# millardjn/rusty_sr

Measured on AMD Instinct MI355X. Metric: output megapixels/sec at 3x upscale (BASELINE '4x'; reference factor is hard-wired 3), higher is better.
Workload: dtype f32; 1 GPU; 1920x1080 RGB x3 upscale per GPU, imagenet.rsr, rgba8 in/out resident in HBM; io=rgba8, factor=3, parallelism=rowband1, precision=f32

## Files before the change

### rusty_sr_amd/csrc/sr_kernels.hip

```cpp
#include <hip/hip_runtime.h>
#include <stddef.h>
#include <stdint.h>

#include <mutex>
#include <set>
#include <type_traits>
#include <utility>

#include "sr_kernels.h"

#pragma clang fp contract(off)

typedef float f32x2 __attribute__((ext_vector_type(2)));
struct f32p { float x, y; };
__device__ __forceinline__ f32p operator+(f32p a, f32p b) { return f32p{a.x + b.x, a.y + b.y}; }
__device__ __forceinline__ f32p operator-(f32p a, f32p b) { return f32p{a.x - b.x, a.y - b.y}; }
__device__ __forceinline__ f32p operator*(f32p a, f32p b) { return f32p{a.x * b.x, a.y * b.y}; }
__device__ __forceinline__ f32p p_fma(f32p a, f32p b, f32p c) { return f32p{__builtin_fmaf(a.x, b.x, c.x), __builtin_fmaf(a.y, b.y, c.y)}; }
__device__ __forceinline__ void store_map8(char* p, uint32_t a, uint32_t b) { *(uint2*)p = make_uint2(a, b); }
typedef float f32x4 __attribute__((ext_vector_type(4)));
typedef float f32x16 __attribute__((ext_vector_type(16)));
typedef _Float16 f16x8 __attribute__((ext_vector_type(8)));
typedef _Float16 f16x2 __attribute__((ext_vector_type(2)));

template <int PREC>
constexpr bool kPlanar = PREC == 1;
template <int PREC, bool FINAL>
constexpr bool kH16 = PREC == 1 && !FINAL;

namespace {

constexpr int kThreads = 256;
constexpr int kTW = 32;
constexpr int kChunkFloats = 1024;
constexpr int kRingSlots = 5;
constexpr int kRingAhead = 4;
constexpr int kRingBytes = kRingSlots * 4096;

__device__ __forceinline__ float belu(float v, float beta) {
    return __fadd_rn(__fadd_rn(__fmul_rn(beta, v), __builtin_amdgcn_sqrtf(__fadd_rn(__fmul_rn(v, v), 1.0f))), -1.0f);
}

__device__ __forceinline__ f32x2 belu2(f32x2 v, float beta) {
    const f32x2 one = {1.0f, 1.0f};
    const f32x2 t = v * v + one;
    const f32x2 s = {__builtin_amdgcn_sqrtf(t.x), __builtin_amdgcn_sqrtf(t.y)};
    const f32x2 b = {beta, beta};
    return (b * v + s) - one;
}

__device__ __forceinline__ f32p split_value(f32p accm, f32p accx) {
    return p_fma(accx, f32p{1.0f / 2048.0f, 1.0f / 2048.0f}, accm);
}
__device__ __forceinline__ f32p belu2_fused2(f32p v, f32p beta) {
    const f32p one = {1.0f, 1.0f};
    const f32p t = p_fma(v, v, one);
    const f32p s = {__builtin_amdgcn_sqrtf(t.x), __builtin_amdgcn_sqrtf(t.y)};
    return p_fma(beta, v, s) - one;
}

__device__ __forceinline__ void store_belu_tile(float* base, const f32x16& acc, float bias, float beta) {
#pragma unroll
    for (int r = 0; r < 16; r += 2) {
        const f32x2 bb = {bias, bias};
        const f32x2 o = belu2(f32x2{acc[r], acc[r + 1]} + bb, beta);
        const int row = (r & 3) + 8 * (r >> 2);
        base[row * 32] = o.x;
        base[(row + 1) * 32] = o.y;
    }
}

__device__ __forceinline__ void store_belu_tile_lds(float* grow, float* stage, const f32x16& acc, float bias, float beta, int lane) {
    float* sp = stage + (4 * (lane >> 5)) * 32 + (lane & 31);
#pragma unroll
    for (int r = 0; r < 16; r += 2) {
        const f32x2 bb = {bias, bias};
        const f32x2 o = belu2(f32x2{acc[r], acc[r + 1]} + bb, beta);
        const int row = (r & 3) + 8 * (r >> 2);
        sp[row * 32] = o.x;
        sp[(row + 1) * 32] = o.y;
    }
    const f32x4* lp = (const f32x4*)stage + lane;
    const f32x4 v0 = lp[0], v1 = lp[64], v2 = lp[128], v3 = lp[192];
    f32x4* gp = (f32x4*)grow + lane;
    gp[0] = v0; gp[64] = v1; gp[128] = v2; gp[192] = v3;
}

__device__ __forceinline__ int xcd_remap(int bid, int nblk) {
    const int q = nblk >> 3, r = nblk & 7, xcd = bid & 7, idx = bid >> 3;
    return (xcd < r ? xcd * (q + 1) : r * (q + 1) + (xcd - r) * q) + idx;
}

__device__ __forceinline__ int tile_div(int t, TileDiv d) {
    return (int)((__umulhi((uint32_t)t, d.m) + (uint32_t)t) >> d.s);
}

__device__ __forceinline__ void tile_coords(const TileGrid& g, int tiles_x, int t, int& n, int& tx, int& ty) {
    const int tpi = tiles_x * g.tiles_y;
    n = tile_div(t, g.div_tpi);
    const int r = t - n * tpi;
    if (g.bw == 0) {
        ty = tile_div(r, g.div_tx);
        tx = r - ty * tiles_x;
    } else {
        int b = tile_div(r, g.div_blk);
        if (b > g.nfull) b = g.nfull;
        const int rr = r - b * g.bw * g.tiles_y;
        const bool full = b < g.nfull;
        const int w = full ? g.bw : tiles_x - g.nfull * g.bw;
        ty = full ? tile_div(rr, g.div_bw) : tile_div(rr, g.div_rem);
        tx = b * g.bw + (rr - ty * w);
    }
}

__device__ __forceinline__ float load_img(const void* img, int img_ch, bool u8, size_t px, int c) {
    if (u8) return __fdiv_rn((float)((const uint8_t*)img)[px * img_ch + c], 255.0f);
    return ((const float*)img)[px * 3 + c];
}

constexpr float kLoScale = 2048.0f;
typedef __fp16 fp16x2_t __attribute__((ext_vector_type(2)));

__device__ __forceinline__ void split_half2(f32p v, uint32_t& hi2, uint32_t& lo2) {
    const fp16x2_t h = __builtin_amdgcn_cvt_pkrtz(v.x, v.y);
    const f32p hf = {(float)h.x, (float)h.y};
    const f32p r = (v - hf) * f32p{kLoScale, kLoScale};
    hi2 = __builtin_bit_cast(uint32_t, h);
    lo2 = __builtin_bit_cast(uint32_t, __builtin_amdgcn_cvt_pkrtz(r.x, r.y));
}

typedef unsigned short u16x2 __attribute__((ext_vector_type(2)));
__device__ __forceinline__ void domain_track(uint32_t& dom, uint32_t hi2) {
    dom = __builtin_bit_cast(uint32_t, __builtin_elementwise_max(__builtin_bit_cast(u16x2, dom), __builtin_bit_cast(u16x2, hi2 & 0x7fff7fffu)));
}
__device__ __forceinline__ void domain_report(uint32_t dom, int* flag) {
    if (((dom & 0xffffu) >= 0x7bffu) | ((dom >> 16) >= 0x7bffu)) *(volatile int*)flag = 1;
}

__device__ __forceinline__ void store_belu_tile_split_cr(char* base, const f32x16& accm, const f32x16& accx, const f32x4 (&beta)[4], bool write,
                                                         long group_stride, long lo_off, uint32_t& dom) {
#pragma unroll
    for (int j = 0; j < 4; ++j) {
        const int r = 4 * j;
        const f32p v01 = belu2_fused2(split_value(f32p{accm[r], accm[r + 1]}, f32p{accx[r], accx[r + 1]}), f32p{beta[j][0], beta[j][1]});
        const f32p v23 = belu2_fused2(split_value(f32p{accm[r + 2], accm[r + 3]}, f32p{accx[r + 2], accx[r + 3]}), f32p{beta[j][2], beta[j][3]});
        uint32_t h01, l01, h23, l23;
        split_half2(v01, h01, l01);
        split_half2(v23, h23, l23);
        domain_track(dom, h01);
        domain_track(dom, h23);
        if (write) {
            store_map8(base + j * group_stride, h01, h23);
            store_map8(base + j * group_stride + lo_off, l01, l23);
        }
    }
}

template <typename F>
__device__ __forceinline__ void for_each_acc_row(F&& f) {
#pragma unroll
    for (int r = 0; r < 16; ++r) f(r, (r & 3) + 8 * (r >> 2));
}

}

__device__ __forceinline__ const char* uniform_ptr(const void* p) {
    const uint64_t v = (uint64_t)(uintptr_t)p;
    const uint32_t lo = __builtin_amdgcn_readfirstlane((uint32_t)v), hi = __builtin_amdgcn_readfirstlane((uint32_t)(v >> 32));
    return (const char*)(uintptr_t)(((uint64_t)hi << 32) | lo);
}

template <int TH, bool IMG_U8>
__global__ __launch_bounds__(kThreads, 2) void conv0_kernel(Conv0Args a) {
    constexpr int T = TH / 4;
    constexpr int TWH = kTW + 4, THH = TH + 4, NPIX = THH * TWH;
    __shared__ __attribute__((aligned(16))) float s_x[NPIX * 3 + 16];
    __shared__ __attribute__((aligned(16))) float s_w[5 * 8 * 64];

    const int tid = threadIdx.x, lane = tid & 63;
    const int wave = __builtin_amdgcn_readfirstlane(tid >> 6);
    const int i = lane & 31, h = lane >> 5;
    const int tiles_per_img = a.tiles_x * a.tiles_y;
    for (int k = tid; k < 5 * 8 * 64; k += kThreads) s_w[k] = a.wpack[k];
    if (tid < 16) s_x[NPIX * 3 + tid] = 0.f;
    if (blockIdx.x == 0 && tid < 40) a.queue_reset[tid] = (a.queue_grid[tid >> 3] - (tid & 7) + 7) >> 3;
    __shared__ float s_lut[256];
    if constexpr (IMG_U8) s_lut[tid] = __fdiv_rn((float)tid, 255.0f);
    const float bias = a.bias[i], beta = a.beta[i];
  for (int bid = blockIdx.x; bid < a.n_tiles; bid += gridDim.x) {
    const int n = tile_div(bid, a.div_tpi), t = bid - n * tiles_per_img;
    const int ty = tile_div(t, a.div_tx), tx = t - ty * a.tiles_x;
    const int x0 = tx * kTW, y0 = a.y_begin + ty * TH;
    const size_t img_px0 = (size_t)n * a.H * a.W;

    __syncthreads();
    for (int p = tid; p < NPIX; p += kThreads) {
        const int py = p / TWH, px = p - py * TWH;
        const int gy = y0 - 2 + py, gx = x0 - 2 + px;
        f32x4 v = {0.f, 0.f, 0.f, 0.f};
        if (gy >= 0 && gy < a.H && gx >= 0 && gx < a.W) {
            const size_t gp = img_px0 + (size_t)gy * a.W + gx;
            if constexpr (IMG_U8) {
                const uint8_t* q = (const uint8_t*)a.img + gp * a.img_ch;
                v.x = s_lut[q[0]]; v.y = s_lut[q[1]]; v.z = s_lut[q[2]];
            } else {
                v.x = load_img(a.img, a.img_ch, false, gp, 0);
                v.y = load_img(a.img, a.img_ch, false, gp, 1);
                v.z = load_img(a.img, a.img_ch, false, gp, 2);
            }
        }
        s_x[p * 3] = v.x; s_x[p * 3 + 1] = v.y; s_x[p * 3 + 2] = v.z;
    }
    __syncthreads();

    f32x16 acc[T];
#pragma unroll
    for (int m = 0; m < T; ++m)
#pragma unroll
        for (int r = 0; r < 16; ++r) acc[m][r] = 0.f;

    const float* xa = s_x + ((wave * T) * TWH + i) * 3 + h;
    const float* wb = s_w + (h * 32 + i) * 2;
#pragma unroll
    for (int ky = 0; ky < 5; ++ky) {
#pragma unroll
        for (int jj = 0; jj < 4; ++jj) {
            const f32x2 b = *(const f32x2*)(wb + (ky * 4 + jj) * 128);
#pragma unroll
            for (int m = 0; m < T; ++m) {
                const float* row = xa + (m + ky) * TWH * 3;
                acc[m] = __builtin_amdgcn_mfma_f32_32x32x2f32(row[4 * jj], b.x, acc[m], 0, 0, 0);
                const float a2 = (jj == 3 && h) ? 0.0f : row[4 * jj + 2];
                acc[m] = __builtin_amdgcn_mfma_f32_32x32x2f32(a2, b.y, acc[m], 0, 0, 0);
            }
        }
    }

    const bool full_x = x0 + kTW <= a.W;
#pragma unroll
    for (int m = 0; m < T; ++m) {
        const int y = y0 + wave * T + m;
        if (y >= a.y_end) continue;
        float* base = a.dst + ((size_t)n * a.img_stride + (long)y * a.pitch + x0 + 4 * h) * 32 + i;
        if (full_x) {
            store_belu_tile(base, acc[m], bias, beta);
        } else {
            for_each_acc_row([&](int r, int row) {
                if (x0 + 4 * h + row < a.W) base[row * 32] = belu(__fadd_rn(acc[m][r], bias), beta);
            });
        }
    }
  }
}

template <int TH, bool IMG_U8>
__global__ __launch_bounds__(kThreads, 3) void conv0_split_kernel(Conv0Args a) {
    constexpr int T = TH / 4;
    constexpr int TWH = kTW + 4, THH = TH + 4, NPIX = THH * TWH;
    constexpr int NB = 7;
    __shared__ __attribute__((aligned(16))) uint32_t s_px[2][NPIX * 2];
    __shared__ uint32_t s_lut[256];
    const int tid = threadIdx.x, lane = tid & 63;
    const int wave = __builtin_amdgcn_readfirstlane(tid >> 6);
    const int i = lane & 31, h = lane >> 5;
    const int tiles_per_img = a.tiles_x * a.tiles_y;
    if (blockIdx.x == 0 && tid < 40) a.queue_reset[tid] = (a.queue_grid[tid >> 3] - (tid & 7) + 7) >> 3;
    if constexpr (IMG_U8) {
        uint32_t hi2, lo2;
        split_half2(f32p{__fdiv_rn((float)tid, 255.0f), 0.0f}, hi2, lo2);
        s_lut[tid] = (hi2 & 0xffffu) | (lo2 << 16);
    }
    __shared__ __attribute__((aligned(16))) f16x8 s_w[NB * 2 * 64];
    for (int k = tid; k < NB * 2 * 64; k += kThreads) s_w[k] = ((const f16x8*)a.wpack_split)[k];
    const f16x8* wl = s_w + h * 32 + i;
    uint32_t off_a[NB], off_b[NB];
#pragma unroll
    for (int b = 0; b < NB; ++b) {
        const int ta = min(4 * b + 2 * h, 24), tb = min(4 * b + 2 * h + 1, 24);
        off_a[b] = (uint32_t)(((ta / 5) * TWH + ta % 5) * 8);
        off_b[b] = (uint32_t)(((tb / 5) * TWH + tb % 5) * 8);
    }
    const char* abase = (const char*)&s_px[0][0] + ((wave * T) * TWH + i) * 8;
    constexpr uint32_t LO = NPIX * 2 * 4;
    f32x4 bias4[4], beta4[4];
#pragma unroll
    for (int j = 0; j < 4; ++j) {
        bias4[j] = *(const f32x4*)(a.bias + 8 * j + 4 * h);
        beta4[j] = *(const f32x4*)(a.beta + 8 * j + 4 * h);
    }
    uint32_t dom = 0;
    for (int bid = blockIdx.x; bid < a.n_tiles; bid += gridDim.x) {
        const int n = tile_div(bid, a.div_tpi), t = bid - n * tiles_per_img;
        const int ty = tile_div(t, a.div_tx), tx = t - ty * a.tiles_x;
        const int x0 = tx * kTW, y0 = a.y_begin + ty * TH;
        const size_t img_px0 = (size_t)n * a.H * a.W;
        __syncthreads();
        for (int p = tid; p < NPIX; p += kThreads) {
            const int py = p / TWH, px = p - py * TWH;
            const int gy = y0 - 2 + py, gx = x0 - 2 + px;
            uint32_t h0 = 0, h1 = 0, l0 = 0, l1 = 0;
            if (gy >= 0 && gy < a.H && gx >= 0 && gx < a.W) {
                const size_t gp = img_px0 + (size_t)gy * a.W + gx;
                if constexpr (IMG_U8) {
                    const uint8_t* q = (const uint8_t*)a.img + gp * a.img_ch;
                    const uint32_t wr = s_lut[q[0]], wg = s_lut[q[1]], wb = s_lut[q[2]];
                    h0 = __builtin_amdgcn_perm(wg, wr, 0x05040100u); l0 = __builtin_amdgcn_perm(wg, wr, 0x07060302u);
                    h1 = wb & 0xffffu; l1 = wb >> 16;
                } else {
                    const float* q = (const float*)a.img + gp * 3;
                    split_half2(f32p{q[0], q[1]}, h0, l0);
                    split_half2(f32p{q[2], 0.0f}, h1, l1);
                    domain_track(dom, h0);
                    domain_track(dom, h1);
                }
            }
            *(uint2*)&s_px[0][p * 2] = make_uint2(h0, h1);
            *(uint2*)&s_px[1][p * 2] = make_uint2(l0, l1);
        }
        __syncthreads();

        f32x16 accm[T], accx[T];
#pragma unroll
        for (int m = 0; m < T; ++m)
#pragma unroll
            for (int r = 0; r < 16; ++r) { accm[m][r] = bias4[r >> 2][r & 3]; accx[m][r] = 0.f; }
#pragma unroll
        for (int b = 0; b < NB; ++b) {
            const f16x8 bh = wl[(b * 2 + 0) * 64], bl = wl[(b * 2 + 1) * 64];
#pragma unroll
            for (int m = 0; m < T; ++m) {
                const char* ra = abase + off_a[b] + m * TWH * 8;
                const char* rb = abase + off_b[b] + m * TWH * 8;
                const uint2 ha = *(const uint2*)ra, hb2 = *(const uint2*)rb;
                const uint2 la = *(const uint2*)(ra + LO), lb2 = *(const uint2*)(rb + LO);
                const uint32_t ahw[4] = {ha.x, ha.y, hb2.x, hb2.y}, alw[4] = {la.x, la.y, lb2.x, lb2.y};
                const f16x8 ah = __builtin_bit_cast(f16x8, ahw), al = __builtin_bit_cast(f16x8, alw);
                accm[m] = __builtin_amdgcn_mfma_f32_32x32x16_f16(bh, ah, accm[m], 0, 0, 0);
                accx[m] = __builtin_amdgcn_mfma_f32_32x32x16_f16(bl, ah, accx[m], 0, 0, 0);
                accx[m] = __builtin_amdgcn_mfma_f32_32x32x16_f16(bh, al, accx[m], 0, 0, 0);
            }
        }

        const bool full_x = x0 + kTW <= a.W;
#pragma unroll
        for (int m = 0; m < T; ++m) {
            const int y = y0 + wave * T + m;
            if (y >= a.y_end) continue;
            char* base = (char*)(a.dst + ((size_t)n * a.img_stride + (long)y * a.pitch) * 32) + (size_t)(x0 + i) * 16 + 8 * h;
            store_belu_tile_split_cr(base, accm[m], accx[m], beta4, full_x || x0 + i < a.W, (long)a.pitch * 16, (long)a.pitch * 64, dom);
        }
    }
    domain_report(dom, a.domain);
}

template <int TH, int KS>
struct TileGeom {
    static constexpr int R = KS / 2;
    static constexpr int TWH = kTW + 2 * R;
    static constexpr int THH = TH + 2 * R;
    static constexpr int NPIX = THH * TWH;
    static constexpr int NG = (NPIX + 63) / 64;
    static constexpr int PLANE = NG * 64 * 16;
};

template <int IMM>
__device__ __forceinline__ void lds_dma16(const void* base, uint32_t voff, uint32_t lds) {
    asm volatile("s_mov_b32 m0, %0\n\ts_nop 3\n\tglobal_load_lds_dwordx4 %1, %2 offset:%3"
                 :: "s"(lds), "v"(voff), "s"(base), "n"(IMM) : "memory");
}
__device__ __forceinline__ void lds_dma16_at(const void* base, uint32_t byte_off, uint32_t voff, uint32_t lds) {
    const uint64_t b = (uint64_t)(uintptr_t)base;
    asm volatile("s_add_u32 vcc_lo, %0, %2\n\ts_addc_u32 vcc_hi, %1, 0\n\ts_mov_b32 m0, %3\n\ts_nop 0\n\tglobal_load_lds_dwordx4 %4, vcc offset:0"
                 :: "s"((uint32_t)b), "s"((uint32_t)(b >> 32)), "s"(__builtin_amdgcn_readfirstlane(byte_off)), "s"(__builtin_amdgcn_readfirstlane(lds)), "v"(voff)
                 : "vcc", "scc", "memory");
}
__device__ __forceinline__ uint32_t lds_addr(const void* p) {
    return (uint32_t)(uintptr_t)(const __attribute__((address_space(3))) char*)p;
}

template <int TH, int KS, int NW = 4>
struct TileOffsets {
    using G = TileGeom<TH, KS>;
    static constexpr int N = (G::NG + NW - 1) / NW;
    uint32_t v[N];
    template <int PREC>
    __device__ __forceinline__ void init(int pitch, int wave, int lane) {
#pragma unroll
        for (int gi = 0; gi < N; ++gi) {
            const int P = min((wave + NW * gi) * 64 + lane, G::NPIX - 1);
            const int prow = P / G::TWH, pcol = P - prow * G::TWH;
            v[gi] = kPlanar<PREC> ? (uint32_t)(prow * pitch) * 128u + (uint32_t)pcol * 16u : (uint32_t)(prow * pitch + pcol) * 128u;
        }
    }
};

template <int TH, int KS, int PREC, int NW = 4>
__device__ __forceinline__ void stage_tile(char* tile, const float* __restrict__ src, const TileOffsets<TH, KS, NW>& off,
                                           long img_stride, int pitch, int n, int y0, int x0, int wave, int ) {
    using G = TileGeom<TH, KS>;
    const char* origin = kPlanar<PREC> ? uniform_ptr((const char*)(src + ((size_t)n * img_stride + (long)(y0 - G::R) * pitch) * 32) + (long)(x0 - G::R) * 16)
                                       : uniform_ptr(src + ((size_t)n * img_stride + (long)(y0 - G::R) * pitch + (x0 - G::R)) * 32);
#pragma unroll
    for (int gi = 0; gi < TileOffsets<TH, KS, NW>::N; ++gi) {
        const int g = wave + NW * gi;
        if (g < G::NG) {
            const uint32_t dst = __builtin_amdgcn_readfirstlane(lds_addr(tile) + g * 1024);
            if constexpr (kPlanar<PREC>) {
#pragma unroll
                for (int c = 0; c < 8; ++c) lds_dma16_at(origin, (uint32_t)(c * pitch * 16), off.v[gi], dst + c * G::PLANE);
            } else {
#define SR_DMA16(c) lds_dma16<(c) * 16>(origin, off.v[gi], dst + (c) * (G::PLANE - 16))
                SR_DMA16(0); SR_DMA16(1); SR_DMA16(2); SR_DMA16(3); SR_DMA16(4); SR_DMA16(5); SR_DMA16(6); SR_DMA16(7);
#undef SR_DMA16
            }
        }
    }
}

__device__ __forceinline__ void weight_chunk_async(char* ring_slot, const float* __restrict__ chunk,
                                                   int wave, int lane) {
    lds_dma16<0>(uniform_ptr((const char*)chunk + wave * 1024), (uint32_t)(lane * 16),
                 __builtin_amdgcn_readfirstlane(lds_addr(ring_slot) + wave * 1024));
}

template <int PENDING>
__device__ __forceinline__ void ring_barrier() {
    static_assert(PENDING >= 0 && PENDING <= 3, "");
    if constexpr (PENDING == 3) asm volatile("s_waitcnt vmcnt(3) lgkmcnt(0)" ::: "memory");
    else if constexpr (PENDING == 2) asm volatile("s_waitcnt vmcnt(2) lgkmcnt(0)" ::: "memory");
    else if constexpr (PENDING == 1) asm volatile("s_waitcnt vmcnt(1) lgkmcnt(0)" ::: "memory");
    else asm volatile("s_waitcnt vmcnt(0) lgkmcnt(0)" ::: "memory");
    __builtin_amdgcn_s_barrier();
    asm volatile("" ::: "memory");
}

__device__ __forceinline__ void ring_request(char* ring, const float* __restrict__ wpack, int gtap, int slot,
                                             int ntaps_total, int wave, int lane) {
    if (gtap + kRingAhead < ntaps_total) {
        int s2 = slot + kRingAhead;
        if (s2 >= kRingSlots) s2 -= kRingSlots;
        weight_chunk_async(ring + s2 * 4096, wpack + (size_t)(gtap + kRingAhead) * kChunkFloats, wave, lane);
    }
}
template <int EXTRA = 0>
__device__ __forceinline__ void ring_advance(int& gtap, int& slot, int ntaps_total) {
    const int pending = max(0, min(kRingAhead - 1 - EXTRA, ntaps_total - 2 - EXTRA - gtap));
    ++gtap;
    slot = slot == kRingSlots - 1 ? 0 : slot + 1;
    if (pending >= 3) ring_barrier<3>();
    else if (pending == 2) ring_barrier<2>();
    else if (pending == 1) ring_barrier<1>();
    else ring_barrier<0>();
}

template <int ABID>
__device__ __forceinline__ f32x4 mfma_quad(float w, float p, f32x4 c) { return __builtin_amdgcn_mfma_f32_4x4x1f32(w, p, c, 4, ABID, 0); }
template <int FACTOR>
constexpr int quad_groups(int nt) {
    const int ntr = FACTOR * FACTOR - 10 * nt < 10 ? FACTOR * FACTOR - 10 * nt : 10, tl = ntr - 1;
    return (16 * (tl / 5) + 3 * (tl % 5) + 2) / 4 + 1;
}
typedef f32x4 QuadAcc[8];
template <int H, int NG>
__device__ __forceinline__ void quad_rank1(QuadAcc& acc, float w, float p) {
    if constexpr (NG > 0) acc[0] = mfma_quad<8 * H + 0>(w, p, acc[0]);
    if constexpr (NG > 1) acc[1] = mfma_quad<8 * H + 1>(w, p, acc[1]);
    if constexpr (NG > 2) acc[2] = mfma_quad<8 * H + 2>(w, p, acc[2]);
    if constexpr (NG > 3) acc[3] = mfma_quad<8 * H + 3>(w, p, acc[3]);
    if constexpr (NG > 4) acc[4] = mfma_quad<8 * H + 4>(w, p, acc[4]);
    if constexpr (NG > 5) acc[5] = mfma_quad<8 * H + 5>(w, p, acc[5]);
    if constexpr (NG > 6) acc[6] = mfma_quad<8 * H + 6>(w, p, acc[6]);
    if constexpr (NG > 7) acc[7] = mfma_quad<8 * H + 7>(w, p, acc[7]);
}
template <int FACTOR, int H>
__device__ __forceinline__ void quad_rank1_tile(QuadAcc& acc, int nt, float w, float p) {
    if (nt == 0) quad_rank1<H, quad_groups<FACTOR>(0)>(acc, w, p);
    else quad_rank1<H, quad_groups<FACTOR>(1)>(acc, w, p);
}

template <int TWH, int PS, int KS, int T, int NTN, bool QUAD = false, int FACTOR = 3, typename Acc, typename Stream>
__device__ __forceinline__ void half_steps_f32(Acc& acc, const char* hb, const char* ring, Stream& sm, int wave, int lane) {
    constexpr int NT = KS * KS, NP = (NT + 1) / 2;
    static_assert(!QUAD || T == 2, "the quad form: 64 pixels = two tile rows per wave");
    const int i = lane & 31, h = lane >> 5;
    const int wlane = (h * 32 + i) * 16;
    const char* abase = QUAD ? hb + ((wave * T + h) * TWH + i) * 16 : hb + h * PS + ((wave * T) * TWH + i) * 16;
    struct Ops { f32x4 a[T]; f32x4 b; };
    auto load = [&](Ops& o, int p, int q, int sl) {
        const int t = 2 * p + (q >> 1), ky = t / KS, kx = t - ky * KS;
        const char* ab = abase + (q & 1) * 2 * PS + (ky * TWH + kx) * 16;
        o.b = *(const f32x4*)(ring + sl * 4096 + wlane + q * 1024);
#pragma unroll
        for (int m = 0; m < T; ++m) o.a[m] = *(const f32x4*)(ab + (QUAD ? m * PS : m * TWH * 16));
    };
    auto mfma = [&](const Ops& o, int nt) {
        if constexpr (QUAD) {
#pragma unroll
            for (int e = 0; e < 4; ++e) {
                quad_rank1_tile<FACTOR, 0>(acc[nt], nt, o.b[e], o.a[0][e]);
                quad_rank1_tile<FACTOR, 1>(acc[nt], nt, o.b[e], o.a[1][e]);
            }
        } else {
#pragma unroll
            for (int e = 0; e < 4; ++e)
#pragma unroll
                for (int m = 0; m < T; ++m)
                    acc[nt * T + m] = __builtin_amdgcn_mfma_f32_32x32x2f32(o.a[m][e], o.b[e], acc[nt * T + m], 0, 0, 0);
        }
    };
    Ops cur, nxt;
    load(cur, 0, 0, sm.slot());
#pragma unroll
    for (int p = 0; p < NP; ++p) {
#pragma unroll
      for (int nt = 0; nt < NTN; ++nt) {
        const int ngroups = (2 * p + 1 < NT) ? 4 : 2;
        sm.begin_step();
#pragma unroll
        for (int q = 0; q < 3; ++q) {
            if (q + 1 < ngroups) {
                load(nxt, p, q + 1, sm.slot());
                if (((p * NTN + nt) * 4 + q) % NTN == 0) sm.piece(((p * NTN + nt) * 4 + q) / NTN);
                __builtin_amdgcn_sched_barrier(0);
                mfma(cur, nt);
                __builtin_amdgcn_sched_barrier(0);
                cur = nxt;
            }
        }
        const bool last = p == NP - 1 && nt == NTN - 1;
        sm.template end_step<0>(last);
        if (!last) load(nxt, nt + 1 < NTN ? p : p + 1, 0, sm.slot());
        if (((p * NTN + nt) * 4 + 3) % NTN == 0) sm.piece(((p * NTN + nt) * 4 + 3) / NTN);
        __builtin_amdgcn_sched_barrier(0);
        mfma(cur, nt);
        __builtin_amdgcn_sched_barrier(0);
        cur = nxt;
      }
    }
}

constexpr int wino_positions(int ks) { return ks == 5 ? 7 : 4; }
constexpr int wino_groups(int ks) { return ks * wino_positions(ks) * 2; }
constexpr int wino_steps(int ks) { return (wino_groups(ks) + 3) / 4; }
constexpr int kWinoSteps = wino_steps(5), kWino3Steps = wino_steps(3);
constexpr int wino_acc(int k) { return k < 4 ? k : k - 3; }
constexpr int wino_ca(int k) { return k == 0 ? 0 : k == 1 ? 1 : k == 2 ? 2 : k == 3 ? 1 : k == 4 ? 3 : k == 5 ? 4 : 3; }
constexpr int wino_cb(int k) { return k == 0 ? 2 : k == 1 ? 2 : k == 2 ? 1 : k == 3 ? 3 : k == 4 ? 4 : k == 5 ? 3 : 5; }
constexpr bool wino_add(int k) { return k == 1 || k == 4; }

template <bool ADD>
__device__ __forceinline__ void wino_u4(f32x2 x0, f32x2 y0, f32x2 x1, f32x2 y1, f32x2& u0, f32x2& u1) {
    if constexpr (ADD)
        asm("v_pk_add_f32 %0, %2, %3\n\tv_pk_add_f32 %1, %4, %5\n\ts_nop 1"
            : "=&v"(u0), "=&v"(u1) : "v"(x0), "v"(y0), "v"(x1), "v"(y1));
    else
        asm("v_pk_add_f32 %0, %2, %3 neg_lo:[0,1] neg_hi:[0,1]\n\tv_pk_add_f32 %1, %4, %5 neg_lo:[0,1] neg_hi:[0,1]\n\ts_nop 1"
            : "=&v"(u0), "=&v"(u1) : "v"(x0), "v"(y0), "v"(x1), "v"(y1));
}

template <int TWH, int PS, int T, int KS, int NA, typename Stream>
__device__ __forceinline__ void half_steps_wino(f32x16 (&acc)[NA], const char* hb, const char* ring, Stream& sm, int wave, int lane) {
    static_assert(KS == 5 || KS == 3, "5-tap rows: chunks A and B; 3-tap rows: chunk A");
    static_assert(TWH >= kTW + KS - 1, "a pair reads KS + 1 pixels from its first halo column on: the highest is column 2 * 15 + KS");
    constexpr int NPOS = wino_positions(KS), NGROUPS = wino_groups(KS), NSTEPS = wino_steps(KS);
    const int i = lane & 31, h = lane >> 5;
    const int wlane = (h * 32 + i) * 16;
    const int row = wave * T + (T == 2 ? i >> 4 : 0);
    const char* abase = hb + h * PS + (row * TWH + 2 * (i & 15)) * 16;
    struct Ops { f32x4 x, y, b; };
    auto load = [&](Ops& o, int g, int sl) {
        const int rr = g & 1, k = (g >> 1) % NPOS, ky = (g >> 1) / NPOS;
        const char* ab = abase + rr * 2 * PS + ky * TWH * 16;
        o.b = *(const f32x4*)(ring + sl * 4096 + wlane + (g & 3) * 1024);
        o.x = *(const f32x4*)(ab + wino_ca(k) * 16);
        o.y = *(const f32x4*)(ab + wino_cb(k) * 16);
    };
    auto mfma = [&](const Ops& o, int g) {
        const int k = (g >> 1) % NPOS;
        const f32x2 x0 = {o.x[0], o.x[1]}, x1 = {o.x[2], o.x[3]}, y0 = {o.y[0], o.y[1]}, y1 = {o.y[2], o.y[3]};
        f32x2 u0, u1;
        if (wino_add(k)) wino_u4<true>(x0, y0, x1, y1, u0, u1);
        else wino_u4<false>(x0, y0, x1, y1, u0, u1);
        const float u[4] = {u0.x, u0.y, u1.x, u1.y};
#pragma unroll
        for (int e = 0; e < 4; ++e) acc[wino_acc(k)] = __builtin_amdgcn_mfma_f32_32x32x2f32(u[e], o.b[e], acc[wino_acc(k)], 0, 0, 0);
    };
    Ops cur, nxt;
    load(cur, 0, sm.slot());
#pragma unroll
    for (int s = 0; s < NSTEPS; ++s) {
        const int ngroups = NGROUPS - 4 * s < 4 ? NGROUPS - 4 * s : 4;
        sm.begin_step();
#pragma unroll
        for (int q = 0; q < 3; ++q) {
            if (q + 1 < ngroups) {
                load(nxt, 4 * s + q + 1, sm.slot());
                sm.piece(4 * s + q);
                __builtin_amdgcn_sched_barrier(0);
                mfma(cur, 4 * s + q);
                __builtin_amdgcn_sched_barrier(0);
                cur = nxt;
            }
        }
        const bool last = s == NSTEPS - 1;
        sm.template end_step<0>(last);
        if (!last) load(nxt, 4 * s + 4, sm.slot());
        sm.piece(4 * s + 3);
        __builtin_amdgcn_sched_barrier(0);
        mfma(cur, 4 * s + ngroups - 1);
        __builtin_amdgcn_sched_barrier(0);
        cur = nxt;
    }
}

template <int TWH, int PS, int T, typename Stream>
__device__ __forceinline__ void half_steps_pairs(f32x16 (&acc)[5], const char* hb, const char* ring, Stream& sm, int wave, int lane) {
    constexpr int NT = 9, NP = (NT + 1) / 2;
    static_assert(TWH >= kTW + 2, "a pair reads four pixels from its first halo column on");
    const int i = lane & 31, h = lane >> 5;
    const int wlane = (h * 32 + i) * 16;
    const int row = wave * T + (T == 2 ? i >> 4 : 0);
    const char* abase = hb + h * PS + (row * TWH + 2 * (i & 15)) * 16;
    struct Ops { f32x4 x, y, b; };
    auto load = [&](Ops& o, int p, int q, int sl) {
        const int t = 2 * p + (q >> 1), ky = t / 3, kx = t - ky * 3;
        const char* ab = abase + (q & 1) * 2 * PS + (ky * TWH + kx) * 16;
        o.b = *(const f32x4*)(ring + sl * 4096 + wlane + q * 1024);
        o.x = *(const f32x4*)ab;
        o.y = *(const f32x4*)(ab + 16);
    };
    auto mfma = [&](const Ops& o) {
#pragma unroll
        for (int e = 0; e < 4; ++e) {
            acc[0] = __builtin_amdgcn_mfma_f32_32x32x2f32(o.x[e], o.b[e], acc[0], 0, 0, 0);
            acc[4] = __builtin_amdgcn_mfma_f32_32x32x2f32(o.y[e], o.b[e], acc[4], 0, 0, 0);
        }
    };
    Ops cur, nxt;
    load(cur, 0, 0, sm.slot());
#pragma unroll
    for (int p = 0; p < NP; ++p) {
        const int ngroups = (2 * p + 1 < NT) ? 4 : 2;
        sm.begin_step();
#pragma unroll
        for (int q = 0; q < 3; ++q) {
            if (q + 1 < ngroups) {
                load(nxt, p, q + 1, sm.slot());
                sm.piece(4 * p + q);
                __builtin_amdgcn_sched_barrier(0);
                mfma(cur);
                __builtin_amdgcn_sched_barrier(0);
                cur = nxt;
            }
// ... 1515 lines not shown
```

Baseline: 5303 output MP/s.

## Double-buffer conv0 input tile staging with register prefetch of next tile

The first-layer conv kernel now keeps two LDS buffers for the haloed input tile. Each thread issues global loads for the next tile into registers before the current tile's MFMA work, then writes them into the alternate buffer after the MFMAs. This is meant to hide global load latency behind compute and to drop one barrier per tile. Per-thread pixel coordinates are precomputed, and u8 pixels are fetched as a single 4-byte load with a guard for the final pixel. In exchange, LDS use doubles and register pressure rises, which may lower occupancy.

```diff
diff --git a/rusty_sr_amd/csrc/sr_kernels.hip b/rusty_sr_amd/csrc/sr_kernels.hip
--- a/rusty_sr_amd/csrc/sr_kernels.hip
+++ b/rusty_sr_amd/csrc/sr_kernels.hip
@@ -258,7 +258,9 @@
     constexpr int T = TH / 4;
     constexpr int TWH = kTW + 4, THH = TH + 4, NPIX = THH * TWH;
     constexpr int NB = 7;
-    __shared__ __attribute__((aligned(16))) uint32_t s_px[2][NPIX * 2];
+    constexpr int NP = (NPIX + kThreads - 1) / kThreads;
+    static_assert(NP == 2 && NPIX > kThreads, "a thread stages one or two pixels of the haloed tile");
+    __shared__ __attribute__((aligned(16))) uint32_t s_px[2][2][NPIX * 2];
     __shared__ uint32_t s_lut[256];
     const int tid = threadIdx.x, lane = tid & 63;
     const int wave = __builtin_amdgcn_readfirstlane(tid >> 6);
@@ -280,57 +282,115 @@
         off_a[b] = (uint32_t)(((ta / 5) * TWH + ta % 5) * 8);
         off_b[b] = (uint32_t)(((tb / 5) * TWH + tb % 5) * 8);
     }
-    const char* abase = (const char*)&s_px[0][0] + ((wave * T) * TWH + i) * 8;
+    const char* abase = (const char*)&s_px[0][0][0] + ((wave * T) * TWH + i) * 8;
     constexpr uint32_t LO = NPIX * 2 * 4;
+    constexpr uint32_t BUF = 2 * LO;
     f32x4 bias4[4], beta4[4];
 #pragma unroll
     for (int j = 0; j < 4; ++j) {
         bias4[j] = *(const f32x4*)(a.bias + 8 * j + 4 * h);
         beta4[j] = *(const f32x4*)(a.beta + 8 * j + 4 * h);
     }
-    uint32_t dom = 0;
-    for (int bid = blockIdx.x; bid < a.n_tiles; bid += gridDim.x) {
+    const uint32_t esz = IMG_U8 ? (uint32_t)a.img_ch : 12u;
+    int ppy[NP], ppx[NP];
+    uint32_t slot[NP], rel[NP];
+#pragma unroll
+    for (int k = 0; k < NP; ++k) {
+        const int p = tid + k * kThreads;
+        const int py = p / TWH;
+        ppy[k] = p < NPIX ? py : (1 << 30);
+        ppx[k] = p - py * TWH;
+        slot[k] = (uint32_t)p * 8u;
+        rel[k] = ((uint32_t)py * (uint32_t)a.W + (uint32_t)ppx[k]) * esz;
+    }
+    const bool second = tid < NPIX - kThreads;
+    const long total_px = (long)(a.n_tiles / tiles_per_img) * a.H * a.W;
+    struct TileAt { int n, x0, y0; };
+    auto tile_at = [&](int bid) {
         const int n = tile_div(bid, a.div_tpi), t = bid - n * tiles_per_img;
         const int ty = tile_div(t, a.div_tx), tx = t - ty * a.tiles_x;
-        const int x0 = tx * kTW, y0 = a.y_begin + ty * TH;
-        const size_t img_px0 = (size_t)n * a.H * a.W;
+        return TileAt{n, tx * kTW, a.y_begin + ty * TH};
+    };
+    struct RawF32 { float r, g, b; };
+    using Raw = typename std::conditional<IMG_U8, uint32_t, RawF32>::type;
+    auto request = [&](const TileAt& t, Raw (&raw)[NP]) {
+        const long org = ((long)t.n * a.H + (t.y0 - 2)) * a.W + (t.x0 - 2);
+        const char* tb = (const char*)a.img + org * (long)esz;
+        uint32_t last_rel = 0xffffffffu;
+        if constexpr (IMG_U8) {
+            const long d = (total_px - 1 - org) * (long)esz;
+            if (a.img_ch < 4 && d >= 0 && d < 0xffffffffL) last_rel = (uint32_t)d;
+        }
+#pragma unroll
+        for (int k = 0; k < NP; ++k) {
+            const uint32_t gy = (uint32_t)(t.y0 - 2 + ppy[k]), gx = (uint32_t)(t.x0 - 2 + ppx[k]);
+            const char* q = tb + rel[k];
+            if constexpr (IMG_U8) {
+                raw[k] = 0u;
+                if (gy < (uint32_t)a.H && gx < (uint32_t)a.W) {
+                    if (rel[k] == last_rel) {
+                        const uint8_t* qb = (const uint8_t*)q;
+                        raw[k] = (uint32_t)qb[0] | ((uint32_t)qb[1] << 8) | ((uint32_t)qb[2] << 16);
+                    } else {
+                        __builtin_memcpy(&raw[k], q, 4);
+                    }
+                }
+            } else {
+                raw[k] = RawF32{0.0f, 0.0f, 0.0f};
+                if (gy < (uint32_t)a.H && gx < (uint32_t)a.W) __builtin_memcpy(&raw[k], q, 12);
+            }
+        }
+    };
+    uint32_t dom = 0;
+    auto stage = [&](const Raw (&raw)[NP], uint32_t buf) {
+#pragma unroll
+        for (int k = 0; k < NP; ++k) {
+            if (k > 0 && !second) continue;
+            uint32_t h0, h1, l0, l1;
+            if constexpr (IMG_U8) {
+                const uint32_t wr = s_lut[raw[k] & 0xffu], wg = s_lut[(raw[k] >> 8) & 0xffu], wb = s_lut[(raw[k] >> 16) & 0xffu];
+                h0 = __builtin_amdgcn_perm(wg, wr, 0x05040100u); l0 = __builtin_amdgcn_perm(wg, wr, 0x07060302u);
+                h1 = wb & 0xffffu; l1 = wb >> 16;
+            } else {
+                split_half2(f32p{raw[k].r, raw[k].g}, h0, l0);
+                split_half2(f32p{raw[k].b, 0.0f}, h1, l1);
+                domain_track(dom, h0);
+                domain_track(dom, h1);
+            }
+            char* d = (char*)&s_px[0][0][0] + buf + slot[k];
+            *(uint2*)d = make_uint2(h0, h1);
+            *(uint2*)(d + LO) = make_uint2(l0, l1);
+        }
+    };
+
+    const int step = (int)gridDim.x;
+    int bid = blockIdx.x;
+    if (bid >= a.n_tiles) return;
+    TileAt cur = tile_at(bid), nxt = cur;
+    Raw raw[NP];
+    request(cur, raw);
+    __syncthreads();
+    stage(raw, 0);
+    if (bid + step < a.n_tiles) {
+        nxt = tile_at(bid + step);
+        request(nxt, raw);
+    }
+    uint32_t buf = 0;
+    for (;; bid += step) {
         __syncthreads();
-        for (int p = tid; p < NPIX; p += kThreads) {
-            const int py = p / TWH, px = p - py * TWH;
-            const int gy = y0 - 2 + py, gx = x0 - 2 + px;
-            uint32_t h0 = 0, h1 = 0, l0 = 0, l1 = 0;
-            if (gy >= 0 && gy < a.H && gx >= 0 && gx < a.W) {
-                const size_t gp = img_px0 + (size_t)gy * a.W + gx;
-                if constexpr (IMG_U8) {
-                    const uint8_t* q = (const uint8_t*)a.img + gp * a.img_ch;
-                    const uint32_t wr = s_lut[q[0]], wg = s_lut[q[1]], wb = s_lut[q[2]];
-                    h0 = __builtin_amdgcn_perm(wg, wr, 0x05040100u); l0 = __builtin_amdgcn_perm(wg, wr, 0x07060302u);
-                    h1 = wb & 0xffffu; l1 = wb >> 16;
-                } else {
-                    const float* q = (const float*)a.img + gp * 3;
-                    split_half2(f32p{q[0], q[1]}, h0, l0);
-                    split_half2(f32p{q[2], 0.0f}, h1, l1);
-                    domain_track(dom, h0);
-                    domain_track(dom, h1);
-                }
-            }
-            *(uint2*)&s_px[0][p * 2] = make_uint2(h0, h1);
-            *(uint2*)&s_px[1][p * 2] = make_uint2(l0, l1);
-        }
-        __syncthreads();
-
         f32x16 accm[T], accx[T];
 #pragma unroll
         for (int m = 0; m < T; ++m)
 #pragma unroll
             for (int r = 0; r < 16; ++r) { accm[m][r] = bias4[r >> 2][r & 3]; accx[m][r] = 0.f; }
+        const char* ab = abase + buf;
 #pragma unroll
         for (int b = 0; b < NB; ++b) {
             const f16x8 bh = wl[(b * 2 + 0) * 64], bl = wl[(b * 2 + 1) * 64];
 #pragma unroll
             for (int m = 0; m < T; ++m) {
-                const char* ra = abase + off_a[b] + m * TWH * 8;
-                const char* rb = abase + off_b[b] + m * TWH * 8;
+                const char* ra = ab + off_a[b] + m * TWH * 8;
+                const char* rb = ab + off_b[b] + m * TWH * 8;
                 const uint2 ha = *(const uint2*)ra, hb2 = *(const uint2*)rb;
                 const uint2 la = *(const uint2*)(ra + LO), lb2 = *(const uint2*)(rb + LO);
                 const uint32_t ahw[4] = {ha.x, ha.y, hb2.x, hb2.y}, alw[4] = {la.x, la.y, lb2.x, lb2.y};
@@ -341,6 +401,17 @@
             }
         }
 
+        const int n = cur.n, x0 = cur.x0, y0 = cur.y0;
+        const bool more = bid + step < a.n_tiles;
+        if (more) {
+            stage(raw, buf ^ BUF);
+            cur = nxt;
+            if (bid + 2 * step < a.n_tiles) {
+                nxt = tile_at(bid + 2 * step);
+                request(nxt, raw);
+            }
+        }
+
         const bool full_x = x0 + kTW <= a.W;
 #pragma unroll
         for (int m = 0; m < T; ++m) {
@@ -349,6 +420,8 @@
             char* base = (char*)(a.dst + ((size_t)n * a.img_stride + (long)y * a.pitch) * 32) + (size_t)(x0 + i) * 16 + 8 * h;
             store_belu_tile_split_cr(base, accm[m], accx[m], beta4, full_x || x0 + i < a.W, (long)a.pitch * 16, (long)a.pitch * 64, dom);
         }
+        if (!more) break;
+        buf ^= BUF;
     }
     domain_report(dom, a.domain);
 }
```

After: 5290 output MP/s. About the same (-0.2%).
